# noahares/raxtax

Hardware: AMD Instinct MI355X
Metric: classified queries/sec (whole node) (higher is better)
Workload: dtype u32 bit-planes + f64

## Files before the change

raxtax_amd/csrc/rtx_emul.cpp:

```cpp
#include <algorithm>
#include <cmath>
#include <cstdint>
#include <cstring>
#include <array>
#include <vector>

#include "rtx_math.hpp"

using namespace rtx;

extern "C" {

uint32_t emul_planes_grouped(const uint32_t *rows, uint32_t n_rows, uint32_t groups, uint32_t *out) {
    constexpr int NP = 10;
    std::vector<std::array<uint32_t, NP>> part(groups);
    for (auto &p : part) p.fill(0);
    for (uint32_t u = 0; u + 8 * groups <= n_rows; u += 8 * groups)
        for (uint32_t g = 0; g < groups; g++) {
            const uint32_t *r = rows + u + 8 * g;
            uint32_t pl[NP];
            for (int p = 0; p < NP; p++) pl[p] = part[g][p];
            planes_ripple<NP, 3>(pl, planes_tree8<NP>(pl, r[0], r[1], r[2], r[3], r[4], r[5], r[6], r[7]));
            for (int p = 0; p < NP; p++) part[g][p] = pl[p];
        }
// ... 445 lines not shown
void emul_prune_threshold(uint32_t t, uint64_t n_refs, const uint32_t *hm_in, const double *lf, uint32_t tab_tmax, uint32_t *u_out,
                          uint32_t *i1_out) {
    emul_prune_threshold_x(t, n_refs, hm_in, lf, tab_tmax, 0, nullptr, nullptr, u_out, i1_out);
}
void emul_prune_threshold_tiles(uint32_t t, uint64_t n_refs, const uint32_t *hm_in, const double *lf, uint32_t tab_tmax, uint32_t ntiles,
                                const uint16_t *tile_ub, uint32_t *u_out, uint32_t *i1_out) {
    const uint32_t per = (ntiles + 63u) / 64u, ng = (ntiles + per - 1u) / per;
    std::vector<uint32_t> gub(ng, 0);
    std::vector<uint64_t> gn(ng, 0);
    for (uint32_t T = 0; T < ntiles; T++) {
        const uint32_t g = T / per;
        gub[g] = std::max<uint32_t>(gub[g], tile_ub[T]);
        const uint64_t lo = (uint64_t)T * 8192u, hi = std::min<uint64_t>(lo + 8192u, n_refs);
        gn[g] += hi > lo ? hi - lo : 0u;
    }
    emul_prune_threshold_x(t, n_refs, hm_in, lf, tab_tmax, ng, gub.data(), gn.data(), u_out, i1_out);
}

void emul_ref_slot(uint32_t r, uint32_t stride_bytes, uint32_t *word, uint32_t *bit) { ref_slot(r, stride_bytes, *word, *bit); }
uint32_t emul_slot_ref(uint32_t tile, uint32_t lane, uint32_t g, uint32_t j, uint32_t stride_bytes) {
    return tile * 8192u + (g * tile_lanes(stride_bytes, tile) + lane) * 8u + j;
}

void emul_merge_bytes(const uint32_t *sb, uint32_t *st) {
    st[0] += (sb[0] & 0xFFu) | ((sb[0] & 0xFF00u) << 8);
    st[1] += ((sb[0] >> 16) & 0xFFu) | ((sb[0] >> 24) << 16);
    st[2] += (sb[1] & 0xFFu) | ((sb[1] & 0xFF00u) << 8);
    st[3] += ((sb[1] >> 16) & 0xFFu) | ((sb[1] >> 24) << 16);
}

void emul_transpose64(const unsigned long long *in, unsigned long long *out) {
    unsigned long long x[64], y[64];
    for (int l = 0; l < 64; l++) x[l] = in[l];
    for (int s = 32; s >= 1; s >>= 1) {
        const unsigned long long m = s == 32 ? 0x00000000FFFFFFFFull : s == 16 ? 0x0000FFFF0000FFFFull : s == 8 ? 0x00FF00FF00FF00FFull
                                   : s == 4 ? 0x0F0F0F0F0F0F0F0Full : s == 2 ? 0x3333333333333333ull : 0x5555555555555555ull;
        for (int l = 0; l < 64; l++) y[l] = x[l ^ s];
        for (int l = 0; l < 64; l++) x[l] = (l & s) ? (((y[l] >> s) & m) | (x[l] & ~m)) : ((x[l] & m) | ((y[l] & m) << s));
    }
    for (int l = 0; l < 64; l++) out[l] = x[l];
}

uint32_t emul_finalise_rows(uint32_t n, uint32_t D, const uint8_t *k, const uint32_t *depth, const uint32_t *size, double n_total, uint32_t *rank,
                            double *local) {
    const uint32_t kw = (D + 3u) / 4u;
    std::vector<uint32_t> words((size_t)n * kw, 0u);
    for (uint32_t r = 0; r < n; r++)
        for (uint32_t w = 0; w < kw; w++) {
            uint32_t v = 0;
            for (uint32_t b = 0; b < 4u; b++) {
                const uint32_t d = 4u * w + b;
                v |= (uint32_t)(d < depth[r] && d < D ? k[(size_t)r * D + d] : 0u) << (8u * b);
            }
            words[(size_t)r * kw + w] = fin_be32(v);
        }
    uint32_t disagree = 0;
    for (uint32_t r = 0; r < n; r++) {
        uint32_t before = 0;
        for (uint32_t x = 0; x < n; x++) {
            const bool a = x != r && fin_row_before(k + (size_t)x * D, depth[x], x, k + (size_t)r * D, depth[r], r);
            const bool b = x != r && fin_row_before_words(&words[(size_t)x * kw], depth[x], x, &words[(size_t)r * kw], depth[r], r, kw);
            disagree += a != b;
            before += b ? 1u : 0u;
        }
        rank[r] = before;
        double eb[64];
        const uint32_t s0 = fin_node_expected(size + (size_t)r * D, depth[r], n_total, eb);
        const uint8_t *kr = k + (size_t)r * D;
        local[r] = fin_local_signal([&](uint32_t d) { return kr[d]; }, eb, s0, depth[r]);
    }
    return disagree;
}

int64_t emul_text_numbers(const double *v, uint64_t n, uint32_t n_hund, char *out, uint64_t cap) {
    TextWindow w{out, 0, 0, cap};
    for (uint64_t i = 0; i < n; i++) { text_put_fix5(w, v[i]); w.put('\n'); }
    for (uint32_t k = 0; k < n_hund; k++) { text_put_hund(w, k); w.put('\n'); }
    return w.pos > cap ? -1 : (int64_t)w.pos;
}

int64_t emul_text_batch(const char *lin_bytes, const uint64_t *lin_off, const uint8_t *lin_depth, const uint32_t *row_lineage,
                        const uint8_t *row_depth, const uint8_t *row_hund, const double *row_local, uint32_t D, uint64_t nq,
                        const char *labels, const uint64_t *label_off, const uint8_t *status, const uint64_t *row_begin,
                        const uint32_t *row_count, const double *gs, const uint32_t *one, const uint8_t *seq, const uint64_t *seq_off,
                        int tsv, char *out, uint64_t cap, uint64_t *out_off) {
    const TextSrc t{lin_bytes, lin_off, lin_depth, row_lineage, row_depth, row_hund, row_local, D};
    TextWindow w{out, 0, 0, cap};
    for (uint64_t q = 0; q < nq; q++) {
        out_off[q] = w.pos;
        const uint64_t n_out = status[q] != 0 || row_count[q] == 0 ? 0 : (one[q] != kTextNoOverride ? 1 : row_count[q]);
        for (uint64_t i = 0; i < n_out; i++) {
            if (i) w.put('\n');
            const TextRow r = text_row(t, labels + label_off[q], label_off[q + 1] - label_off[q], row_begin[q], i, one[q], gs[q]);
            if (tsv) {
                const uint8_t *sq = seq + seq_off[q];
                text_tsv_row(w, r, seq_off[q + 1] - seq_off[q], [&](uint64_t j) { return sq[j]; });
            } else {
                text_out_row(w, r);
            }
        }
        w.put('\0');
    }
    out_off[nq] = w.pos;
    return w.pos > cap ? -1 : (int64_t)w.pos;
}

uint32_t emul_nearest_scan(const void *lo, const uint16_t *hi, uint32_t in_tile, uint32_t peak, int packed) {
    const uint32_t per = packed ? 16u : 8u;
    for (uint32_t step = 0; nearest_lane_base(step, 0u, per) < in_tile; step++) {
        uint32_t mask[64];
        for (uint32_t lane = 0; lane < 64u; lane++) {
            const uint32_t b0 = nearest_lane_base(step, lane, per);
            mask[lane] = 0;
            if (b0 >= in_tile) continue;
            uint32_t w[4];
            if (packed) {
                std::memcpy(w, static_cast<const uint8_t *>(lo) + b0, 16);
                uint32_t h2;
                std::memcpy(&h2, hi + (b0 >> 3), 4);
                mask[lane] = nearest_match16(w, h2, peak, b0, in_tile);
            } else {
                std::memcpy(w, static_cast<const uint16_t *>(lo) + b0, 16);
                mask[lane] = nearest_match8(w, peak, b0, in_tile);
            }
        }
        for (uint32_t lane = 0; lane < 64u; lane++)
            if (mask[lane]) return nearest_lane_base(step, lane, per) + (uint32_t)__builtin_ctz(mask[lane]);
    }
    return 0xFFFFFFFFu;
}
void emul_packed_count_pos(uint32_t rl, uint32_t *byte, uint32_t *hi_word, uint32_t *hi_shift) { packed_count_pos(rl, *byte, *hi_word, *hi_shift); }

void emul_profile(uint64_t nq, const uint8_t *status, const uint32_t *row_count, const uint64_t *row_begin, const uint32_t *row_node,
                  const uint8_t *row_depth, const uint8_t *row_hund, uint32_t D, const uint32_t *parent, const uint8_t *node_depth,
                  const uint32_t *ref_leaf, uint32_t n_nodes, uint32_t n_refs, const uint32_t *one, uint32_t cutoff, uint64_t *clade,
                  uint64_t *direct, uint64_t *conf_sum, uint64_t *totals) {
    const ProfileSrc src{status, row_count, reinterpret_cast<const unsigned long long *>(row_begin), row_node, row_depth, row_hund, D, parent, node_depth, ref_leaf, n_nodes, n_refs};
    for (uint64_t q = 0; q < nq; q++) {
        const ProfileStep st = profile_step(src, q, one[q], cutoff);
        totals[0]++;
        totals[st.kind == kProfClassified ? 1 : (st.kind == kProfUnclassified ? 2 : 3)]++;
        if (st.kind != kProfClassified) continue;
        uint32_t node = st.node;
        for (uint32_t d = st.L; d-- > 0u;) {
            if (node >= n_nodes) break;
            clade[node]++;
            conf_sum[node] += st.at(d);
            if (d + 1u == st.L) direct[node]++;
            node = parent[node];
        }
    }
}

}
```

raxtax_amd/csrc/rtx_math.hpp:

```cpp
#pragma once

#include <cmath>
#include <cstdint>

#if defined(__HIPCC__)
#define RTX_HD __host__ __device__ __forceinline__
#else
#define RTX_HD inline
#endif

namespace rtx {


RTX_HD uint32_t tile_lanes(uint32_t stride_bytes, uint32_t tile) {
    const uint32_t rem = stride_bytes - tile * 1024u;
    return rem >= 1024u ? 64u : rem >> 4;
}
RTX_HD size_t bitmap_word(uint32_t row, uint32_t word, uint32_t n_rows1) {
    return ((size_t)(word >> 8) * n_rows1 + row) * 256u + (word & 255u);
}
RTX_HD void ref_slot(uint32_t r, uint32_t stride_bytes, uint32_t &word, uint32_t &bit) {
    const uint32_t tile = r >> 13, rl = r & 8191u;
    const uint32_t L = tile_lanes(stride_bytes, tile);
    const uint32_t c = rl >> 3, l = c % L, g = c / L;
// ... 185 lines not shown
        hi1 |= spread4(pl[p] >> (8 * b + 4)) << (p - 8);
    }
}

RTX_HD uint32_t byte_perm(uint32_t hi, uint32_t lo, uint32_t sel) {
#if defined(__HIP_DEVICE_COMPILE__)
    return __builtin_amdgcn_perm(hi, lo, sel);
#else
    const uint64_t v = ((uint64_t)hi << 32) | lo;
    uint32_t r = 0;
    for (int k = 0; k < 4; k++) {
        const uint32_t s = (sel >> (8 * k)) & 0xFFu;
        if (s < 8u) r |= (uint32_t)((v >> (8 * s)) & 0xFFu) << (8 * k);
    }
    return r;
#endif
}

RTX_HD void delta_swap_regs(uint32_t &a, uint32_t &b, int s, uint32_t m) {
    const uint32_t na = (a & m) | ((b & m) << s), nb = ((a >> s) & m) | (b & ~m);
    a = na;
    b = nb;
}
template <int NP>
RTX_HD void planes_unpack32(const uint32_t (&pl)[NP], uint32_t (&lo)[4][2]) {
    static_assert(NP >= 8, "at least eight planes");
    uint32_t r[8];
#pragma unroll
    for (int p = 0; p < 8; p++) r[p] = pl[p];
#pragma unroll
    for (int p = 0; p < 4; p++) delta_swap_regs(r[p], r[p + 4], 4, 0x0F0F0F0Fu);
#pragma unroll
    for (int p = 0; p < 8; p++)
        if (!(p & 2)) delta_swap_regs(r[p], r[p + 2], 2, 0x33333333u);
#pragma unroll
    for (int p = 0; p < 8; p += 2) delta_swap_regs(r[p], r[p + 1], 1, 0x55555555u);
#pragma unroll
    for (int h = 0; h < 2; h++) {
        const uint32_t x0 = byte_perm(r[4 * h + 1], r[4 * h], 0x05010400u), x1 = byte_perm(r[4 * h + 1], r[4 * h], 0x07030602u);
        const uint32_t y0 = byte_perm(r[4 * h + 3], r[4 * h + 2], 0x05010400u), y1 = byte_perm(r[4 * h + 3], r[4 * h + 2], 0x07030602u);
        lo[0][h] = byte_perm(y0, x0, 0x05040100u);
        lo[1][h] = byte_perm(y0, x0, 0x07060302u);
        lo[2][h] = byte_perm(y1, x1, 0x05040100u);
        lo[3][h] = byte_perm(y1, x1, 0x07060302u);
    }
}
template <int NP>
RTX_HD void planes_unpack8_hi(const uint32_t (&pl)[NP], int b, uint32_t &hi0, uint32_t &hi1) {
    hi0 = 0;
    hi1 = 0;
#pragma unroll
    for (int p = 8; p < NP; p++) {
        hi0 |= spread4(pl[p] >> (8 * b)) << (p - 8);
        hi1 |= spread4(pl[p] >> (8 * b + 4)) << (p - 8);
    }
}

struct PmfState {
    double v;
    double c;
    int k;
};

constexpr double kScaleLn = 354.89135644669199;
constexpr double kScaleUp = 1.2676506002282294e30;
constexpr double kScaleDown = 7.458340731200207e-155;

RTX_HD double ln_binom_tab(const double *lf, uint32_t n, uint32_t k) { return lf[n] - lf[k] - lf[n - k]; }

RTX_HD PmfState pmf_start(const double *lf, uint32_t t, uint32_t n, uint32_t m, double ln_total) {
    double x0 = ln_binom_tab(lf, t - m + n - 1, n) - ln_total;
    PmfState s;
    s.k = 0;
    if (x0 < -600.0) {
        s.k = (int)ceil((-600.0 - x0) / kScaleLn);
        x0 += (double)s.k * kScaleLn;
    }
    s.v = exp(x0);
    s.c = s.v;
    return s;
}

RTX_HD double ln_pmf_tab(const double *lf, uint32_t t, uint32_t n, uint32_t m, uint32_t i, double ln_total);
RTX_HD PmfState pmf_start_at(const double *lf, uint32_t t, uint32_t n, uint32_t m, uint32_t i_s, double ln_total) {
    double x0 = ln_pmf_tab(lf, t, n, m, i_s, ln_total);
    PmfState s;
    s.k = 0;
    if (x0 < -600.0) {
        s.k = (int)ceil((-600.0 - x0) / kScaleLn);
        x0 += (double)s.k * kScaleLn;
    }
    s.v = exp(x0);
    s.c = s.v;
    return s;
}

RTX_HD double pow_uint(double c, uint32_t h) {
    double r = 1.0, b = c;
    while (h) {
        if (h & 1u) r *= b;
        b *= b;
        h >>= 1;
    }
    return r;
}

RTX_HD double pmf_cmf_pow(const PmfState &s, uint32_t h) {
    if (s.k > 0 || !(s.c > 0.0)) return 0.0;
    return pow_uint(s.c, h);
}

struct InvDiv {
    RTX_HD double operator[](uint32_t x) const { return 1.0 / (double)x; }
};
template <class Inv>
RTX_HD void pmf_step(PmfState &s, const Inv &inv, uint32_t t, uint32_t n, uint32_t m, uint32_t i) {
    const double ratio = ((double)(m + i - 1) * inv[i]) * ((double)(n - i + 1) * inv[t - m + n - i]);
    s.v *= ratio;
    s.c += s.v;
    if (s.k > 0 && s.v > kScaleUp) {
        s.v *= kScaleDown;
        s.c *= kScaleDown;
        s.k -= 1;
    }
}

RTX_HD double neg_inf() { return -INFINITY; }

RTX_HD double pmf_ln_cmf(const PmfState &s) {
    if (s.k > 0 || !(s.c > 0.0)) return neg_inf();
    return log(s.c);
}

constexpr double kLnNegligibleP = -100.0;
constexpr double kLnTailSkip = -41.446531673892822;

RTX_HD double ln_pmf_tab(const double *lf, uint32_t t, uint32_t n, uint32_t m, uint32_t i, double ln_total) {
    return ln_binom_tab(lf, m + i - 1, i) + ln_binom_tab(lf, t - m + n - i - 1, n - i) - ln_total;
}

RTX_HD bool group_negligible(const double *lf, uint32_t t, uint32_t n, uint32_t m_hi, uint32_t i_lo, double ln_total) {
    if (i_lo == 0) return false;
    const double up = (double)(m_hi + i_lo - 1) * (double)(n - i_lo + 1);
    const double dn = (double)i_lo * (double)(t - m_hi + n - i_lo);
    if (!(up < dn)) return false;
    return log((double)(n - i_lo + 1)) + ln_pmf_tab(lf, t, n, m_hi, i_lo, ln_total) < kLnTailSkip;
}

constexpr double kPruneEpsHD = 1e-10;
constexpr double kPruneLnEpsHD = -23.025850929940457;
constexpr double kPruneHalfEpsHD = 0.5e-10;
constexpr uint32_t kPruneFarGap = 40;
constexpr uint32_t kPruneMaxNear = 12;

template <class WAf, class WBf>
RTX_HD void prune_window_sums(const double *lf, const double *inv, uint32_t t, uint32_t n, uint32_t m, uint32_t i1, double ln_total,
                              WAf wa, WBf wb, double &sa, double &sb) {
    sa = 0.0;
    sb = 0.0;
    const bool ok = m != 0u && m < t;
    const uint32_t ms = ok ? m : 1u;
    double x0 = ln_pmf_tab(lf, t, n, ms, i1, ln_total);
    if (x0 < -700.0) x0 = -700.0;
    double P = ok ? exp(x0) : 0.0;
    for (uint32_t l = 0; l < 64u && i1 + l <= n; l++) {
        sa += P * wa(l);
        sb += P * wb(l);
        const uint32_t i = i1 + l;
        if (i < n) P *= ((double)(ms + i) * inv[i + 1u]) * ((double)(n - i) * inv[t - ms + n - i - 1u]);
    }
}

RTX_HD double only_last_pmf_tab(const double *lf, uint32_t t, uint32_t n, uint32_t m, double ln_total) {
    if (m == t) return 1.0;
    if (m == 0) return 0.0;
    return exp(ln_binom_tab(lf, m + n - 1, n) - ln_total);
}

RTX_HD bool fin_row_before(const uint8_t *kx, uint32_t dx, uint32_t ix, const uint8_t *ky, uint32_t dy, uint32_t iy) {
    const uint32_t n = dx < dy ? dx : dy;
    for (uint32_t d = 0; d < n; d++)
        if (kx[d] != ky[d]) return kx[d] > ky[d];
    if (dx != dy) return dx > dy;
    return ix < iy;
}
RTX_HD bool fin_row_before_words(const uint32_t *kx, uint32_t dx, uint32_t ix, const uint32_t *ky, uint32_t dy, uint32_t iy, uint32_t kw) {
    for (uint32_t w = 0; w < kw; w++)
        if (kx[w] != ky[w]) return kx[w] > ky[w];
    if (dx != dy) return dx > dy;
    return ix < iy;
}
RTX_HD uint32_t fin_be32(uint32_t v) { return (v >> 24) | ((v >> 8) & 0xFF00u) | ((v << 8) & 0xFF0000u) | (v << 24); }

RTX_HD uint32_t fin_node_expected(const uint32_t *size, uint32_t depth, double n_total, double *eb) {
#if defined(__clang__)
#pragma clang fp contract(off)
#endif
    if (depth == 0) return 0;
    uint32_t s0 = depth - 1u;
    for (uint32_t d = 0; d < depth; d++)
        if (1.0 > (double)size[d] / n_total) { s0 = d; break; }
    double b_sum = 0.0;
    for (uint32_t d = s0; d < depth; d++) b_sum += (double)size[d] / n_total;
    for (uint32_t d = 0; d < depth; d++) eb[d] = d < s0 ? 0.0 : ((double)size[d] / n_total) / b_sum;
    return s0;
}
template <class K>
RTX_HD double fin_local_signal(K k, const double *eb, uint32_t s0, uint32_t depth) {
#if defined(__clang__)
#pragma clang fp contract(off)
#endif
    if (depth == 0) return 0.0;
    double a_sum = 0.0;
    for (uint32_t d = s0; d < depth; d++) a_sum += (double)k(d) / 100.0;
    double s = 0.0;
    for (uint32_t d = s0; d < depth; d += 4u) {
        double e[4];
#pragma unroll
        for (uint32_t u = 0; u < 4u; u++) e[u] = d + u < depth ? eb[d + u] : 0.0;
#pragma unroll
        for (uint32_t u = 0; u < 4u; u++) {
            if (d + u < depth) {
                const double x = ((double)k(d + u) / 100.0) / a_sum - e[u];
                const double xx = x * x;
                s = s + xx;
            }
        }
    }
    return sqrt(s);
}

struct TextCount {
    uint64_t pos = 0;
    RTX_HD void put(char) { pos++; }
    template <class F>
    RTX_HD void put_gen(uint64_t n, F) { pos += n; }
};
struct TextWindow {
    char *buf;
    uint64_t pos, w0, w1;
    RTX_HD void put(char c) {
        if (pos >= w0 && pos < w1) buf[pos - w0] = c;
        pos++;
    }
    template <class F>
    RTX_HD void put_gen(uint64_t n, F f) {
        const uint64_t lo = pos > w0 ? pos : w0, hi = pos + n < w1 ? pos + n : w1;
        for (uint64_t i = lo; i < hi; i++) buf[i - w0] = f(i - pos);
        pos += n;
    }
};

template <class S>
RTX_HD void text_put_u64(S &s, uint64_t v) {
    uint32_t nd = 1;
    for (uint64_t p = 10; nd < 20 && v >= p; p *= 10) nd++;
    uint64_t div = 1;
    for (uint32_t i = 1; i < nd; i++) div *= 10;
    for (uint32_t i = 0; i < nd; i++) {
        s.put((char)('0' + v / div % 10));
        div /= 10;
    }
}

template <class S>
RTX_HD void text_put_big_int(S &s, double v) {
    int e2 = 0;
    const double fr = frexp(v, &e2);
    uint64_t m = (uint64_t)ldexp(fr, 53);
    const int sh = e2 - 53;
    uint32_t limb[34] = {0};
    const int w = sh / 32, b = sh % 32;
    limb[w] = (uint32_t)(m << b);
    limb[w + 1] = (uint32_t)(m >> (32 - b));
    limb[w + 2] = b ? (uint32_t)(m >> (64 - b)) : 0u;
    uint32_t chunk[40];
    int nc = 0, top = 33;
    while (top >= 0) {
        while (top >= 0 && limb[top] == 0) top--;
        if (top < 0) break;
        uint64_t rem = 0;
        for (int i = top; i >= 0; i--) {
            const uint64_t cur = rem << 32 | limb[i];
            limb[i] = (uint32_t)(cur / 1000000000u);
            rem = cur % 1000000000u;
        }
        chunk[nc++] = (uint32_t)rem;
    }
    text_put_u64(s, chunk[nc - 1]);
    for (int i = nc - 2; i >= 0; i--)
        for (uint32_t d = 100000000u; d; d /= 10) s.put((char)('0' + chunk[i] / d % 10));
}

template <class S>
RTX_HD void text_put_fix5(S &s, double v) {
    const bool neg = std::signbit(v);
    if (std::isnan(v)) { if (neg) s.put('-'); s.put('n'); s.put('a'); s.put('n'); return; }
    if (neg) s.put('-');
    if (std::isinf(v)) { s.put('i'); s.put('n'); s.put('f'); return; }
    const double a = fabs(v);
    double I = floor(a);
    const double F = a - I;
    const double p = F * 1e5, e = fma(F, 1e5, -p);
    const double n = floor(p), f = p - n;
    bool up = false;
    if (f >= 0.25) {
// ... 150 lines not shown
```

raxtax_amd/csrc/rtx_prune.hip:

```cpp
#include <hip/hip_runtime.h>

#include "rtx_kernels.hpp"
#include "rtx_math.hpp"
#include "rtx_wave.hpp"

namespace rtx {

static constexpr double kPruneLnEps = kPruneLnEpsHD;
static constexpr double kPruneHalfEps = kPruneHalfEpsHD;
#ifndef RTX_PRUNE_WAVES
#define RTX_PRUNE_WAVES 4
#endif
#ifndef RTX_PRUNE_TURNS
#define RTX_PRUNE_TURNS 16
#endif
static constexpr uint32_t kPruneWavesPerBlock = 4;

__device__ __forceinline__ uint32_t wave_max_u32p(uint32_t v) { return wave_max_u32(v); }

__global__ __launch_bounds__(64 * kPruneWavesPerBlock, RTX_PRUNE_WAVES) void prune_kernel(PruneParams p, ProbTables tb) {
    extern __shared__ double prune_lds[];
    for (uint32_t i = threadIdx.x; i < p.nlf; i += 64u * kPruneWavesPerBlock) prune_lds[i] = p.lnfact[i];
    __syncthreads();
    const uint32_t lane = threadIdx.x & 63u, pair = blockIdx.x * kPruneWavesPerBlock + (threadIdx.x >> 6);
    if (pair * 2u >= p.nq) return;
    uint16_t *ub_lds = reinterpret_cast<uint16_t *>(prune_lds + p.nlf) + (size_t)(threadIdx.x >> 6) * 2u * p.ntiles;
    const double *lf = prune_lds;
    const double ln_n = log((double)p.n_total);
    uint32_t thr[2] = {0u, 0u};
    uint32_t ist_prev = 0;
    unsigned long long st[8] = {0, 0, 0, 0, 0, 0, 0, 0};
    const bool has_b = pair * 2u + 1u < p.nq;
    for (uint32_t x = 0; x < 2u; x++) {
        if (x == 1u && !has_b) break;
        const uint32_t q = pair * 2u + x;
        for (uint32_t T = lane; T < p.ntiles; T += 64) ub_lds[x * p.ntiles + T] = p.tile_ub[(size_t)q * p.tile_ub_stride + T];
        const uint32_t bkey = p.best_key[q];
        uint32_t ub_best = bkey >> 20;
        const uint32_t bb = 0xFFFFFu - (bkey & 0xFFFFFu);
        uint32_t M = 0;
        uint32_t hm = 0;
        if (p.phase == 2u) {
            const uint32_t *bq = p.best + (size_t)q * kPruneBestWords;
            ub_best = bq[0];
            hm = bq[2u + lane];
            M = wave_max_u32p(hm);
        } else if (p.cbitmap) {
            static_assert(kPruneShift == 6, "a block of the block-major bitmap is the block of the bounds");
            const uint32_t nr = p.nrows[q];
            const uint32_t *rows = p.rows + (size_t)q * p.rstride;
            const uint32_t zero_row = p.n_rows1 - 1u;
            const uint32_t nr_pad = (nr + 63u) & ~63u;
            const uint2 *C = p.cbitmap + (size_t)bb * p.n_rows1;
            uint32_t pl[2][11];
#pragma unroll
            for (int w = 0; w < 2; w++)
#pragma unroll
                for (int b = 0; b < 11; b++) pl[w][b] = 0;
            for (uint32_t i0 = 0; i0 < nr_pad; i0 += 256u) {
                uint32_t id[4];
                uint2 v[4];
#pragma unroll
                for (int k = 0; k < 4; k++) {
                    const uint32_t i = i0 + (uint32_t)k * 64u + lane;
                    id[k] = i < nr_pad ? rows[i] : zero_row;
                }
#pragma unroll
                for (int k = 0; k < 4; k++) v[k] = C[id[k]];
#pragma unroll
                for (int k = 0; k < 4; k++) {
                    uint32_t cx = v[k].x, cy = v[k].y;
#pragma unroll
                    for (int b = 0; b < 6; b++) {
                        const uint32_t nx = pl[0][b] & cx, ny = pl[1][b] & cy;
                        pl[0][b] ^= cx;
                        pl[1][b] ^= cy;
                        cx = nx;
                        cy = ny;
                    }
                }
            }
            uint32_t r[11];
            {
                const bool up = (lane & 32u) != 0u;
                uint32_t o[11];
#pragma unroll
                for (int b = 0; b < 11; b++) {
                    r[b] = up ? pl[1][b] : pl[0][b];
                    o[b] = (uint32_t)__shfl_xor((int)(up ? pl[0][b] : pl[1][b]), 32, 64);
                }
                planes_add<11>(r, o);
            }
#pragma unroll
            for (int d = 16; d >= 1; d >>= 1) {
                uint32_t o[11];
#pragma unroll
                for (int b = 0; b < 11; b++) o[b] = (uint32_t)__shfl_xor((int)r[b], d, 64);
                planes_add<11>(r, o);
            }
            uint32_t cnt = 0;
#pragma unroll
            for (int b = 0; b < 11; b++) cnt |= ((r[b] >> (lane & 31u)) & 1u) << b;
            const uint64_t rr = ((uint64_t)bb << kPruneShift) + (uint64_t)lane;
            bool ok = rr < p.n_refs;
            if (p.flags & RTX_SKIP_EXACT_MATCHES) {
                const uint64_t qin = p.perm[p.q0 + q];
                uint64_t xe0 = 0, xe1 = 0;
                const uint32_t *xids = nullptr;
                exact_range(p.exact, qin, xe0, xe1, xids);
                for (uint64_t e = xe0; e < xe1; e++) ok = ok && (uint64_t)(xids[e] - p.ref_base) != rr;
            }
            hm = ok ? cnt : 0u;
            M = wave_max_u32p(hm);
        } else {
            constexpr uint32_t kChunks = (1u << kPruneShift) / 8u;
            const uint32_t nr = p.nrows[q];
            const uint32_t *rows = p.rows + (size_t)q * p.rstride;
            const uint64_t qin = p.perm[p.q0 + q];
            uint64_t xe0 = 0, xe1 = 0;
            const uint32_t *xids = nullptr;
            if (p.flags & RTX_SKIP_EXACT_MATCHES) exact_range(p.exact, qin, xe0, xe1, xids);
            const uint32_t zero_row = p.n_rows1 - 1u;
            constexpr uint32_t kRowsPerTurn = 64u / kChunks;
            const uint32_t ch = lane & (kChunks - 1u), rg = lane / kChunks;
            uint32_t word, bit;
            {
                const uint64_t r0 = ((uint64_t)bb << kPruneShift) + (uint64_t)ch * 8u;
                ref_slot((uint32_t)(r0 < p.n_refs ? r0 : (uint64_t)bb << kPruneShift), p.stride_bytes, word, bit);
            }
            static_assert(kChunks == 8u, "the byte counters of the best block's exact counts hold the rows of one lane in eight (blocks of 64 references)");
            uint32_t acc_lo = 0u, acc_hi = 0u;
            uint32_t acc[4] = {0u, 0u, 0u, 0u};
            const uint32_t bit4 = bit + 4u;
            const uint32_t nr_pad = (nr + 63u) & ~63u;
            constexpr uint32_t kTurns = RTX_PRUNE_TURNS, kPiece = kTurns * kRowsPerTurn;
            static_assert(kPiece % 64u == 0u && kPiece <= 128u, "a piece of the row list = one or two loads per lane");
            auto load_ids = [&](uint32_t i0, uint32_t (&id)[2]) {
#pragma unroll
                for (uint32_t k = 0; k < kPiece / 64u; k++) {
                    const uint32_t i = i0 + k * 64u + lane;
                    id[k] = i < nr_pad ? rows[i] : zero_row;
                }
            };
            uint32_t id[2] = {zero_row, zero_row}, idn[2] = {zero_row, zero_row};
            load_ids(0, id);
            for (uint32_t i0 = 0; i0 < nr; i0 += kPiece) {
                if (i0 + kPiece < nr) load_ids(i0 + kPiece, idn);
                uint32_t w[kTurns];
#pragma unroll
                for (uint32_t u = 0; u < kTurns; u++) {
                    const uint32_t e = u * kRowsPerTurn + rg;
                    const uint32_t row = (uint32_t)__shfl((int)id[e >> 6], (int)(e & 63u), 64);
                    w[u] = p.bitmap[bitmap_word(row, word, p.n_rows1)];
                }
#pragma unroll
                for (uint32_t u = 0; u < kTurns; u++) {
                    acc_lo += __umul24((w[u] >> bit) & 0xFu, 0x204081u) & 0x01010101u;
                    acc_hi += __umul24((w[u] >> bit4) & 0xFu, 0x204081u) & 0x01010101u;
                }
                id[0] = idn[0];
                id[1] = idn[1];
                acc[0] += (acc_lo & 0xFFu) | ((acc_lo & 0xFF00u) << 8);
                acc[1] += ((acc_lo >> 16) & 0xFFu) | ((acc_lo >> 24) << 16);
                acc[2] += (acc_hi & 0xFFu) | ((acc_hi & 0xFF00u) << 8);
                acc[3] += ((acc_hi >> 16) & 0xFFu) | ((acc_hi >> 24) << 16);
                acc_lo = 0u;
                acc_hi = 0u;
            }
#pragma unroll
            for (int k = 0; k < 4; k++)
#pragma unroll
                for (uint32_t d = 32; d >= kChunks; d >>= 1) acc[k] += (uint32_t)__shfl_xor((int)acc[k], (int)d, 64);
            {
                const uint32_t c = lane >> 3, j = lane & 7u;
                const uint32_t v0 = (uint32_t)__shfl((int)acc[0], (int)c, 64), v1 = (uint32_t)__shfl((int)acc[1], (int)c, 64),
                               v2 = (uint32_t)__shfl((int)acc[2], (int)c, 64), v3 = (uint32_t)__shfl((int)acc[3], (int)c, 64);
                const uint32_t vv = (j & 4u) ? ((j & 2u) ? v3 : v2) : ((j & 2u) ? v1 : v0);
                const uint32_t cnt = (vv >> ((j & 1u) * 16u)) & 0xFFFFu;
                const uint64_t r = ((uint64_t)bb << kPruneShift) + (uint64_t)lane;
                bool ok = lane < (1u << kPruneShift) && r < p.n_refs;
                if (p.flags & RTX_SKIP_EXACT_MATCHES)
                    for (uint64_t e = xe0; e < xe1; e++) ok = ok && (uint64_t)(xids[e] - p.ref_base) != r;
                hm = ok ? cnt : 0u;
                M = wave_max_u32p(hm);
            }
        }
        if (p.detail) p.detail[(size_t)q * kPruneDetailWords + 8u + lane] = hm;
        if (p.phase == 1u) {
            uint32_t *bq = p.best + (size_t)q * kPruneBestWords;
            bq[2u + lane] = hm;
            if (lane == 0) { bq[0] = ub_best; bq[1] = 0u; }
            continue;
        }
        const uint32_t t = p.t[q], n = t >> 1;
        uint32_t u_max = 0, i1_q = 0;
        if (t >= 16u && t <= tb.tmax && M >= 1u && n >= 2u) {
            const double ln_total = ln_binom_tab(lf, t + n - 1, n);
            if (M >= t) {
                uint32_t mine = 0;
                for (uint32_t u = 1u + lane; u < t; u += 64)
                    if (ln_binom_tab(lf, u + n - 1, n) - ln_total + ln_n <= kPruneLnEps) mine = u;
                u_max = wave_max_u32p(mine);
            } else {
                const double *Ct = tb.cmf + tb.off[t];
                if (hm * 5u < M * 4u) hm = 0u;
                const double n_h = (double)__popcll(__ballot(hm != 0u));
                const uint32_t h_min = 0xFFFFFFFFu - wave_max_u32p(hm ? 0xFFFFFFFFu - hm : 0u);
                const double ln_f_lo = log(n_h + (double)p.n_total), ln_f_hi = log(n_h + (double)p.n_total * (double)(n - 1u));
                auto passes = [&](uint32_t i) -> bool {
                    const double v = hm ? Ct[(size_t)hm * (n + 1) + i] : 0.0;
                    const double sum = wave_sum_f64_dpp(v);
                    if (sum + ln_f_hi <= kPruneLnEps) return true;
                    if (sum + ln_f_lo > kPruneLnEps) return false;
                    return sum + log(n_h + (double)p.n_total * (double)(i + 1u)) <= kPruneLnEps;
                };
                uint32_t ist1 = 0;
                if (passes(0u)) {
                    uint32_t g;
                    if (x == 1u && ist_prev) g = ist_prev - 1u;
                    else {
                        const double pm = (double)M / (double)t;
                        const double mu = (double)n * pm, sd = sqrt((double)n * pm * (1.0 - pm) * (double)(t + n) / (double)(t + 1u));
                        const double gg = mu - 6.0 * sd;
                        g = gg > 0.0 ? (uint32_t)gg : 0u;
                    }
                    g = g > n - 2u ? n - 2u : g;
                    uint32_t lo, hi;
                    if (passes(g)) {
                        lo = g;
                        uint32_t step = 1u;
                        while (lo + step <= n - 2u && passes(lo + step)) { lo += step; step <<= 1; }
                        hi = lo + step <= n - 2u ? lo + step : n - 1u;
                    } else {
                        hi = g;
                        uint32_t step = 1u;
                        while (hi > step && !passes(hi - step)) { hi -= step; step <<= 1; }
                        lo = hi > step ? hi - step : 0u;
                    }
                    while (hi - lo > 1u) {
                        const uint32_t mid = (lo + hi) >> 1;
                        if (passes(mid)) lo = mid; else hi = mid;
                    }
                    ist1 = lo + 1u;
                }
                ist_prev = ist1;
                if (ist1) {
                    const uint32_t i1 = ist1;
                    const double ln_len = log((double)(n - i1 + 1u));
                    uint32_t first_fail = h_min;
                    for (uint32_t u = 1u + lane; u < h_min; u += 64) {
                        const double up = (double)(u + i1) * (double)(n - i1), dn = (double)(i1 + 1u) * (double)(t - u + n - i1 - 1u);
                        if (!(up < dn && ln_len + ln_pmf_tab(lf, t, n, u, i1, ln_total) + ln_n <= kPruneLnEps)) first_fail = u < first_fail ? u : first_fail;
                    }
                    first_fail = 0xFFFFFFFFu - wave_max_u32p(0xFFFFFFFFu - first_fail);
                    u_max = first_fail - 1u;
                    i1_q = i1;
                    {
                        const bool tile_aware = p.phase == 0u;
                        uint32_t gub = 0;
                        double gnd = 0.0;
                        {
                            const uint32_t per = (p.ntiles + 63u) >> 6;
                            for (uint32_t k = 0; k < per; k++) {
                                const uint32_t T = lane * per + k;
                                if (T < p.ntiles) {
                                    const uint32_t b = ub_lds[x * p.ntiles + T];
                                    gub = b > gub ? b : gub;
                                    const uint64_t lo = (uint64_t)T * 8192u, hi = lo + 8192u < p.n_refs ? lo + 8192u : p.n_refs;
                                    gnd += (double)(hi - lo);
                                }
                            }
                        }
                        const double kept = tile_aware ? wave_sum_f64_dpp(gub > u_max ? gnd : 0.0) : (double)p.n_total;
                        const double ln_kept = log(kept > 1.0 ? kept : 1.0);
                        const uint32_t iw = i1 + lane;
                        const bool tail_pt = lane == 63u;
                        const bool vi = iw <= n;
                        double lnG = 0.0;
                        unsigned long long hb = __ballot(hm != 0u);
                        const uint32_t iwc = vi ? iw : n;
                        while (hb) {
                            double v[4];
#pragma unroll
                            for (int k = 0; k < 4; k++) {
                                v[k] = 0.0;
                                if (hb) {
                                    const int h = __builtin_ctzll(hb);
                                    hb &= hb - 1ull;
                                    const uint32_t m = (uint32_t)__builtin_amdgcn_readlane((int)hm, h);
                                    v[k] = Ct[(size_t)m * (n + 1) + iwc];
                                }
                            }
#pragma unroll
                            for (int k = 0; k < 4; k++) lnG += v[k];
                        }
                        const double gw = vi && !tail_pt ? exp(lnG) : 0.0;
                        const double ww = vi && !tail_pt ? exp(fmin(0.0, ln_kept + lnG)) : 0.0;
                        const double incl = wave_incl_scan_f64_dpp(ww);
                        const double a_tot = readlane_f64(incl, 63);
                        const double len_tail = vi ? (double)(n - iw + 1u) : 0.0;
                        const double WA = tail_pt ? len_tail * (a_tot + 1.0) : (vi ? incl - ww : 0.0);
                        const double WB = tail_pt ? len_tail : gw;
                        const double nn = (double)p.n_total;
                        const bool has_tail = i1 + 63u <= n;
                        auto sums_at = [&](uint32_t m, double &a, double &b) {
                            const double P = vi && m != 0u ? exp(ln_pmf_tab(lf, t, n, m, iw, ln_total)) : 0.0;
                            a = wave_sum_f64_dpp(P * WA);
                            b = wave_sum_f64_dpp(P * WB);
                        };
                        double gsa = 0.0, gsb = 0.0, far_a = 0.0, far_b = 0.0, n_far = 0.0, mid_a = 0.0, mid_b = 0.0, n_mid = 0.0;
                        bool near = false;
                        if (tile_aware) {
                            const uint32_t m_far = u_max > kPruneFarGap ? u_max - kPruneFarGap : 0u;
                            near = gnd > 0.0 && gub > u_max;
                            const bool mid = gnd > 0.0 && gub > m_far && gub <= u_max;
                            unsigned long long nb = __ballot(near);
                            if ((uint32_t)__popcll(nb) > kPruneMaxNear) {
                                near = gnd > 0.0;
                                const uint32_t gcap = gub < h_min ? gub : h_min - 1u;
                                prune_window_sums(lf, p.inv, t, n, gcap, i1, ln_total, [&](uint32_t l) { return readlane_f64(WA, (int)l); },
                                                  [&](uint32_t l) { return readlane_f64(WB, (int)l); }, gsa, gsb);
                            } else {
                                n_far = wave_sum_f64_dpp(near || mid ? 0.0 : gnd);
                                n_mid = wave_sum_f64_dpp(mid ? gnd : 0.0);
                                if (m_far) sums_at(m_far, far_a, far_b);
                                if (n_mid > 0.0) sums_at(u_max, mid_a, mid_b);
                                while (nb) {
                                    const int g = __builtin_ctzll(nb);
                                    nb &= nb - 1ull;
                                    const uint32_t m = (uint32_t)__builtin_amdgcn_readlane((int)gub, g);
                                    double a, b;
                                    sums_at(m < h_min ? m : h_min - 1u, a, b);
                                    if ((int)lane == g) { gsa = a; gsb = b; }
                                }
                            }
                        }
                        auto crit = [&](uint32_t u) -> bool {
                            bool falling = true;
                            if (has_tail) {
                                const uint32_t j = i1 + 63u;
                                falling = (double)(u + j) * (double)(n - j) < (double)(j + 1u) * (double)(t - u + n - j - 1u);
                            }
                            double a, b;
                            sums_at(u, a, b);
                            if (!tile_aware) return falling && nn * a <= kPruneHalfEps && nn * b <= kPruneHalfEps;
                            const bool dead = gub <= u;
                            return falling && wave_sum_f64_dpp(near ? gnd * (dead ? gsa : a) : 0.0) + n_far * far_a + n_mid * mid_a <= kPruneHalfEps &&
                                   wave_sum_f64_dpp(near ? gnd * (dead ? gsb : b) : 0.0) + n_far * far_b + n_mid * mid_b <= kPruneHalfEps;
                        };
                        uint32_t lo = u_max, hi = h_min - 1u;
                        while (lo < hi) {
                            const uint32_t mid = (lo + hi + 1u) >> 1;
                            if (crit(mid)) lo = mid; else hi = mid - 1u;
                        }
                        u_max = lo;
                    }
                }
            }
        }
        thr[x] = u_max;
        if (lane == 0) { p.thr_out[q] = (uint16_t)u_max; p.i1_out[q] = (uint16_t)(u_max ? i1_q : 0u); }
        if (p.detail && lane == 0) {
            uint32_t *d = p.detail + (size_t)q * kPruneDetailWords;
            d[0] = bb; d[1] = M; d[2] = u_max; d[3] = u_max ? i1_q : 0u; d[4] = ub_best; d[5] = t; d[6] = 0u; d[7] = 0u;
        }
        st[2] += M; st[3] += u_max; st[4] += ub_best; st[5] += 1ull;
        if (ub_best < M) st[6] += 1ull;
    }
    if (p.phase == 1u) return;
    __builtin_amdgcn_fence(__ATOMIC_ACQ_REL, "wavefront");
    __builtin_amdgcn_wave_barrier();
    unsigned long long dead_refs[2] = {0, 0};
    uint32_t n_live = 0, n_qlive = 0;
    uint32_t n_rec[2] = {0u, 0u};
    for (uint32_t T0 = 0; T0 < p.ntiles; T0 += 64) {
        const uint32_t T = T0 + lane;
        bool la = false, lb = false;
        if (T < p.ntiles) {
            la = thr[0] == 0u || (uint32_t)ub_lds[T] > thr[0];
            lb = has_b && (thr[1] == 0u || (uint32_t)ub_lds[p.ntiles + T] > thr[1]);
        }
        const unsigned long long ba = __ballot(la), bb2 = __ballot(lb);
        if (lane == 0) {
            uint32_t *wa = p.live + (size_t)(pair * 2u) * p.live_words, *wb = wa + p.live_words;
            wa[T0 >> 5] = (uint32_t)ba;
            if ((T0 >> 5) + 1u < p.live_words) wa[(T0 >> 5) + 1u] = (uint32_t)(ba >> 32);
            if (has_b) {
                wb[T0 >> 5] = (uint32_t)bb2;
                if ((T0 >> 5) + 1u < p.live_words) wb[(T0 >> 5) + 1u] = (uint32_t)(bb2 >> 32);
            }
        }
        if (T < p.ntiles) {
            const uint64_t lo = (uint64_t)T * 8192u, hi = lo + 8192u < p.n_refs ? lo + 8192u : p.n_refs;
            if (!la) dead_refs[0] += hi - lo;
            if (!lb) dead_refs[1] += hi - lo;
        }
        if (p.rec.nslots) {
            const unsigned long long lt = (1ull << lane) - 1ull;
            const uint32_t ka = n_rec[0] + (uint32_t)__popcll(ba & lt), kb = n_rec[1] + (uint32_t)__popcll(bb2 & lt);
            if (la && ka < kRecMaxSlots) p.rec.slots[(size_t)(pair * 2u) * kRecMaxSlots + ka] = (uint16_t)T;
            if (lb && kb < kRecMaxSlots) p.rec.slots[(size_t)(pair * 2u + 1u) * kRecMaxSlots + kb] = (uint16_t)T;
            n_rec[0] += (uint32_t)__popcll(ba);
            n_rec[1] += (uint32_t)__popcll(bb2);
        }
        n_live += (uint32_t)__popcll(ba | bb2);
        n_qlive += (uint32_t)__popcll(ba) + (uint32_t)__popcll(bb2);
    }
    if (p.rec.nslots) {
        const uint32_t cap = p.rec_max_slots < kRecMaxSlots ? p.rec_max_slots : kRecMaxSlots;
        const bool ra = thr[0] != 0u && n_rec[0] != 0u && n_rec[0] <= cap, rb = has_b && thr[1] != 0u && n_rec[1] != 0u && n_rec[1] <= cap;
        if (lane < kRecMaxSlots) {
            p.rec.cnt[(size_t)(pair * 2u) * kRecMaxSlots + lane] = 0u;
            if (has_b) p.rec.cnt[(size_t)(pair * 2u + 1u) * kRecMaxSlots + lane] = 0u;
        }
        if (lane == 0) {
            p.rec.nslots[pair * 2u] = (uint16_t)(ra ? n_rec[0] : 0u);
            if (has_b) p.rec.nslots[pair * 2u + 1u] = (uint16_t)(rb ? n_rec[1] : 0u);
            if (p.cnt_row) {
                auto row_for = [&](bool records) -> uint32_t {
                    if (records) return 0xFFFFFFFFu;
                    const uint32_t r = atomicAdd(p.cnt_cursor, 1u);
                    if (r < p.cnt_cap) return r;
                    atomicOr(p.flags_out, 4u);
                    return 0xFFFFFFFFu;
                };
                p.cnt_row[pair * 2u] = row_for(ra);
                if (has_b) p.cnt_row[pair * 2u + 1u] = row_for(rb);
            }
        }
    }
#pragma unroll
    for (int d = 32; d >= 1; d >>= 1) { dead_refs[0] += __shfl_xor(dead_refs[0], d, 64); dead_refs[1] += __shfl_xor(dead_refs[1], d, 64); }
    if (lane == 0) {
// ... 41 lines not shown
```

Measured before the change: 13.01 million.

## Process both queries of a pair abreast with batched 8-way threshold search

```diff
diff --git a/raxtax_amd/csrc/rtx_emul.cpp b/raxtax_amd/csrc/rtx_emul.cpp
--- a/raxtax_amd/csrc/rtx_emul.cpp
+++ b/raxtax_amd/csrc/rtx_emul.cpp
@@ -621,4 +621,40 @@
     }
 }
 
-}
+uint32_t emul_batched_search(uint32_t n_max, uint32_t guess, int32_t b, uint32_t *info) {
+    uint32_t rounds = 0, asked = 0, c_min = 0xFFFFFFFFu, c_max = 0, outside = 0;
+    const uint32_t r = batched_search(n_max, guess, [&](const uint32_t (&c)[kSearchK], uint32_t cnt) {
+        uint32_t mask = 0;
+        rounds++;
+        for (uint32_t k = 0; k < cnt; k++) {
+            asked++;
+            c_min = std::min(c_min, c[k]);
+            c_max = std::max(c_max, c[k]);
+            outside += c[k] > n_max;
+            if ((int64_t)c[k] <= (int64_t)b) mask |= 1u << k;
+        }
+        return mask;
+    });
+    info[0] = rounds; info[1] = asked; info[2] = c_min; info[3] = c_max; info[4] = outside;
+    return r;
+}
+uint64_t emul_batched_search_grid(uint32_t n_lo, uint32_t n_hi, uint64_t *worst) {
+    uint64_t bad = 0, runs = 0;
+    uint32_t w_rounds = 0, w_asked = 0;
+    for (uint32_t n_max = n_lo; n_max <= n_hi; n_max++)
+        for (int32_t b = -1; b <= (int32_t)n_max; b++) {
+            const int64_t gs[7] = {0, b, (int64_t)b - 1, (int64_t)b + 1, (int64_t)b - 40, (int64_t)b + 40, (int64_t)n_max};
+            for (int64_t g : gs) {
+                uint32_t info[5];
+                const uint32_t r = emul_batched_search(n_max, (uint32_t)std::max<int64_t>(g, 0), b, info);
+                bad += r != (uint32_t)(b + 1) || info[4] != 0u;
+                w_rounds = std::max(w_rounds, info[0]);
+                w_asked = std::max(w_asked, info[1]);
+                runs++;
+            }
+        }
+    worst[0] = w_rounds; worst[1] = w_asked; worst[2] = runs;
+    return bad;
+}
+
+}
diff --git a/raxtax_amd/csrc/rtx_math.hpp b/raxtax_amd/csrc/rtx_math.hpp
--- a/raxtax_amd/csrc/rtx_math.hpp
+++ b/raxtax_amd/csrc/rtx_math.hpp
@@ -361,6 +361,62 @@
 constexpr double kPruneHalfEpsHD = 0.5e-10;
 constexpr uint32_t kPruneFarGap = 40;
 constexpr uint32_t kPruneMaxNear = 12;
+
+constexpr uint32_t kSearchK = 8;
+struct BatchedSearch {
+    uint32_t lo1;
+    uint32_t hi;
+    uint32_t g;
+    uint32_t n_max;
+    bool first;
+    RTX_HD void start(uint32_t n_max_, uint32_t guess) {
+        lo1 = 0u;
+        hi = n_max_ + 1u;
+        n_max = n_max_;
+        g = guess < n_max_ ? guess : n_max_;
+        first = true;
+    }
+    RTX_HD bool done() const { return lo1 >= hi; }
+    RTX_HD uint32_t result() const { return lo1; }
+    RTX_HD uint32_t candidates(uint32_t (&c)[kSearchK]) const {
+        if (first) {
+            const uint32_t down[3] = {32u, 8u, 2u};
+            c[0] = 0u;
+#pragma unroll
+            for (uint32_t k = 0; k < 3u; k++) {
+                c[1u + k] = g > down[k] ? g - down[k] : 0u;
+                c[7u - k] = n_max - g > down[k] ? g + down[k] : n_max;
+            }
+            c[4] = g;
+            return kSearchK;
+        }
+        const uint32_t m = hi - lo1;
+#pragma unroll
+        for (uint32_t k = 0; k < kSearchK; k++)
+            c[k] = m <= kSearchK ? lo1 + (k < m ? k : m - 1u) : lo1 + ((k + 1u) * (m + 1u)) / (kSearchK + 1u) - 1u;
+        return m <= kSearchK ? m : kSearchK;
+    }
+    RTX_HD void update(const uint32_t (&c)[kSearchK], uint32_t cnt, uint32_t pass_mask) {
+#pragma unroll
+        for (uint32_t k = 0; k < kSearchK; k++) {
+            if (k >= cnt) continue;
+            if ((pass_mask >> k) & 1u) lo1 = c[k] + 1u > lo1 ? c[k] + 1u : lo1;
+            else hi = c[k] < hi ? c[k] : hi;
+        }
+        first = false;
+    }
+};
+template <class F>
+RTX_HD uint32_t batched_search(uint32_t n_max, uint32_t guess, F passes_many) {
+    BatchedSearch s;
+    s.start(n_max, guess);
+    while (!s.done()) {
+        uint32_t c[kSearchK];
+        const uint32_t cnt = s.candidates(c);
+        s.update(c, cnt, passes_many(c, cnt));
+    }
+    return s.result();
+}
 
 template <class WAf, class WBf>
 RTX_HD void prune_window_sums(const double *lf, const double *inv, uint32_t t, uint32_t n, uint32_t m, uint32_t i1, double ln_total,
diff --git a/raxtax_amd/csrc/rtx_prune.hip b/raxtax_amd/csrc/rtx_prune.hip
--- a/raxtax_amd/csrc/rtx_prune.hip
+++ b/raxtax_amd/csrc/rtx_prune.hip
@@ -11,12 +11,55 @@
 #ifndef RTX_PRUNE_WAVES
 #define RTX_PRUNE_WAVES 4
 #endif
+#ifndef RTX_PRUNE_ABREAST
+#define RTX_PRUNE_ABREAST 7
+#endif
 #ifndef RTX_PRUNE_TURNS
 #define RTX_PRUNE_TURNS 16
 #endif
+#ifndef RTX_PRUNE_WINDOW_ROWS
+#define RTX_PRUNE_WINDOW_ROWS 16
+#endif
+static constexpr int kWinRows = RTX_PRUNE_WINDOW_ROWS;
 static constexpr uint32_t kPruneWavesPerBlock = 4;
 
 __device__ __forceinline__ uint32_t wave_max_u32p(uint32_t v) { return wave_max_u32(v); }
+
+__device__ __forceinline__ uint32_t block_planes_reduce(const uint32_t (&pl)[2][11], uint32_t lane) {
+    uint32_t r[11];
+    {
+        const bool up = (lane & 32u) != 0u;
+        uint32_t o[11];
+#pragma unroll
+        for (int b = 0; b < 11; b++) {
+            r[b] = up ? pl[1][b] : pl[0][b];
+            o[b] = (uint32_t)__shfl_xor((int)(up ? pl[0][b] : pl[1][b]), 32, 64);
+        }
+        planes_add<11>(r, o);
+    }
+#pragma unroll
+    for (int d = 16; d >= 1; d >>= 1) {
+        uint32_t o[11];
+#pragma unroll
+        for (int b = 0; b < 11; b++) o[b] = (uint32_t)__shfl_xor((int)r[b], d, 64);
+        planes_add<11>(r, o);
+    }
+    uint32_t cnt = 0;
+#pragma unroll
+    for (int b = 0; b < 11; b++) cnt |= ((r[b] >> (lane & 31u)) & 1u) << b;
+    return cnt;
+}
+__device__ __forceinline__ void block_planes_add_row(uint32_t (&pl)[2][11], uint2 v) {
+    uint32_t cx = v.x, cy = v.y;
+#pragma unroll
+    for (int b = 0; b < 6; b++) {
+        const uint32_t nx = pl[0][b] & cx, ny = pl[1][b] & cy;
+        pl[0][b] ^= cx;
+        pl[1][b] ^= cy;
+        cx = nx;
+        cy = ny;
+    }
+}
 
 __global__ __launch_bounds__(64 * kPruneWavesPerBlock, RTX_PRUNE_WAVES) void prune_kernel(PruneParams p, ProbTables tb) {
     extern __shared__ double prune_lds[];
@@ -31,16 +74,216 @@
     uint32_t ist_prev = 0;
     unsigned long long st[8] = {0, 0, 0, 0, 0, 0, 0, 0};
     const bool has_b = pair * 2u + 1u < p.nq;
+#if RTX_PRUNE_ABREAST
+    const bool abreast = p.phase == 0u && p.cbitmap != nullptr;
+#else
+    const bool abreast = false;
+#endif
+    uint32_t pre_hm0 = 0u, pre_hm1 = 0u;
+    uint32_t pre_M[2] = {0u, 0u}, pre_ub[2] = {0u, 0u}, pre_bb[2] = {0u, 0u}, pre_ist1[2] = {0u, 0u};
+    double pre_lnG0 = 0.0, pre_lnG1 = 0.0;
+    if (abreast) {
+        static_assert(kPruneShift == 6, "a block of the block-major bitmap is the block of the bounds");
+        const bool val[2] = {true, has_b};
+        const uint32_t zero_row = p.n_rows1 - 1u;
+        uint32_t tq[2], nr_pad[2];
+        uint64_t toff[2];
+        const uint32_t *rows[2];
+        const uint2 *C[2];
+#pragma unroll
+        for (uint32_t x = 0; x < 2u; x++) {
+            const uint32_t q = pair * 2u + x;
+            uint32_t bkey = 0xFFFFFu, nr = 0u;
+            tq[x] = 0u;
+            if (val[x]) {
+                for (uint32_t T = lane; T < p.ntiles; T += 64) ub_lds[x * p.ntiles + T] = p.tile_ub[(size_t)q * p.tile_ub_stride + T];
+                bkey = p.best_key[q];
+                nr = p.nrows[q];
+                tq[x] = p.t[q];
+            }
+            toff[x] = tq[x] >= 16u && tq[x] <= tb.tmax ? tb.off[tq[x]] : 0ull;
+            pre_ub[x] = bkey >> 20;
+            pre_bb[x] = 0xFFFFFu - (bkey & 0xFFFFFu);
+            nr_pad[x] = (nr + 63u) & ~63u;
+            rows[x] = p.rows + (size_t)(val[x] ? q : pair * 2u) * p.rstride;
+            C[x] = p.cbitmap + (size_t)pre_bb[x] * p.n_rows1;
+        }
+        uint32_t pl[2][2][11];
+#pragma unroll
+        for (int x = 0; x < 2; x++)
+#pragma unroll
+            for (int w = 0; w < 2; w++)
+#pragma unroll
+                for (int b = 0; b < 11; b++) pl[x][w][b] = 0;
+#if RTX_PRUNE_ABREAST & 4
+        const uint32_t pad_max = nr_pad[0] > nr_pad[1] ? nr_pad[0] : nr_pad[1];
+        for (uint32_t i0 = 0; i0 < pad_max; i0 += 256u) {
+            uint32_t id[2][4];
+            uint2 v[2][4];
+#pragma unroll
+            for (int x = 0; x < 2; x++)
+#pragma unroll
+                for (int k = 0; k < 4; k++) {
+                    const uint32_t i = i0 + (uint32_t)k * 64u + lane;
+                    id[x][k] = i < nr_pad[x] ? rows[x][i] : zero_row;
+                }
+#pragma unroll
+            for (int x = 0; x < 2; x++)
+#pragma unroll
+                for (int k = 0; k < 4; k++) v[x][k] = C[x][id[x][k]];
+#pragma unroll
+            for (int x = 0; x < 2; x++)
+#pragma unroll
+                for (int k = 0; k < 4; k++) block_planes_add_row(pl[x], v[x][k]);
+        }
+#else
+#pragma unroll
+        for (int x = 0; x < 2; x++)
+            for (uint32_t i0 = 0; i0 < nr_pad[x]; i0 += 256u) {
+                uint32_t id[4];
+                uint2 v[4];
+#pragma unroll
+                for (int k = 0; k < 4; k++) {
+                    const uint32_t i = i0 + (uint32_t)k * 64u + lane;
+                    id[k] = i < nr_pad[x] ? rows[x][i] : zero_row;
+                }
+#pragma unroll
+                for (int k = 0; k < 4; k++) v[k] = C[x][id[k]];
+#pragma unroll
+                for (int k = 0; k < 4; k++) block_planes_add_row(pl[x], v[k]);
+            }
+#endif
+        uint32_t hmq[2] = {0u, 0u};
+#pragma unroll
+        for (uint32_t x = 0; x < 2u; x++) {
+            if (!val[x]) continue;
+            const uint32_t q = pair * 2u + x;
+            const uint32_t cnt = block_planes_reduce(pl[x], lane);
+            const uint64_t rr = ((uint64_t)pre_bb[x] << kPruneShift) + (uint64_t)lane;
+            bool ok = rr < p.n_refs;
+            if (p.flags & RTX_SKIP_EXACT_MATCHES) {
+                const uint64_t qin = p.perm[p.q0 + q];
+                uint64_t xe0 = 0, xe1 = 0;
+                const uint32_t *xids = nullptr;
+                exact_range(p.exact, qin, xe0, xe1, xids);
+                for (uint64_t e = xe0; e < xe1; e++) ok = ok && (uint64_t)(xids[e] - p.ref_base) != rr;
+            }
+            hmq[x] = ok ? cnt : 0u;
+            pre_M[x] = wave_max_u32p(hmq[x]);
+        }
+        pre_hm0 = hmq[0];
+        pre_hm1 = hmq[1];
+        BatchedSearch sr[2];
+        bool run[2] = {false, false};
+        const double *Ct[2] = {tb.cmf, tb.cmf};
+        uint32_t hmH[2] = {0u, 0u}, nn1[2] = {1u, 1u};
+        double n_h[2] = {0.0, 0.0}, ln_f_lo[2] = {0.0, 0.0}, ln_f_hi[2] = {0.0, 0.0};
+#pragma unroll
+        for (uint32_t x = 0; x < 2u; x++) {
+            const uint32_t t = tq[x], n = t >> 1, M = pre_M[x];
+            if (!(val[x] && t >= 16u && t <= tb.tmax && M >= 1u && n >= 2u && M < t)) continue;
+            Ct[x] = tb.cmf + toff[x];
+            nn1[x] = n + 1u;
+            hmH[x] = hmq[x] * 5u < M * 4u ? 0u : hmq[x];
+            n_h[x] = (double)__popcll(__ballot(hmH[x] != 0u));
+            ln_f_lo[x] = log(n_h[x] + (double)p.n_total);
+            ln_f_hi[x] = log(n_h[x] + (double)p.n_total * (double)(n - 1u));
+            const double pm = (double)M / (double)t;
+            const double mu = (double)n * pm, sd = sqrt((double)n * pm * (1.0 - pm) * (double)(t + n) / (double)(t + 1u));
+            const double gg = mu - 6.0 * sd;
+            sr[x].start(n - 2u, gg > 0.0 ? (uint32_t)gg : 0u);
+            run[x] = true;
+        }
+        while ((run[0] && !sr[0].done()) || (run[1] && !sr[1].done())) {
+            uint32_t c[2][kSearchK], cnt[2] = {0u, 0u};
+            double v[2][kSearchK];
+#pragma unroll
+            for (uint32_t x = 0; x < 2u; x++) {
+                if (!(run[x] && !sr[x].done())) continue;
+                cnt[x] = sr[x].candidates(c[x]);
+                const double *row = Ct[x] + (size_t)hmH[x] * nn1[x];
+#pragma unroll
+                for (uint32_t k = 0; k < kSearchK; k++) v[x][k] = k < cnt[x] && hmH[x] ? row[c[x][k]] : 0.0;
+            }
+#pragma unroll
+            for (uint32_t x = 0; x < 2u; x++) {
+                if (!cnt[x]) continue;
+                uint32_t mask = 0u, band = 0u, cv = 0u;
+                double sv = 0.0;
+#pragma unroll
+                for (uint32_t k = 0; k < kSearchK; k++) {
+                    if (k >= cnt[x]) continue;
+                    const double sum = wave_sum_f64_dpp(v[x][k]);
+                    const bool yes = sum + ln_f_hi[x] <= kPruneLnEps, no = sum + ln_f_lo[x] > kPruneLnEps;
+                    mask |= yes ? 1u << k : 0u;
+                    band |= yes || no ? 0u : 1u << k;
+                    sv = lane == k ? sum : sv;
+                    cv = lane == k ? c[x][k] : cv;
+                }
+                band = (uint32_t)__builtin_amdgcn_readfirstlane((int)band);
+                while (band) {
+                    const int k = __builtin_ctz(band);
+                    band &= band - 1u;
+                    const double sum = readlane_f64(sv, k);
+                    const uint32_t i = (uint32_t)__builtin_amdgcn_readlane((int)cv, k);
+                    if (sum + log(n_h[x] + (double)p.n_total * (double)(i + 1u)) <= kPruneLnEps) mask |= 1u << k;
+                }
+                sr[x].update(c[x], cnt[x], (uint32_t)__builtin_amdgcn_readfirstlane((int)mask));
+            }
+        }
+#pragma unroll
+        for (uint32_t x = 0; x < 2u; x++) pre_ist1[x] = run[x] ? sr[x].result() : 0u;
+#if RTX_PRUNE_ABREAST & 2
+        {
+            unsigned long long hb[2];
+            uint32_t iwc[2];
+            double lnG[2] = {0.0, 0.0};
+#pragma unroll
+            for (uint32_t x = 0; x < 2u; x++) {
+                const uint32_t n = nn1[x] - 1u, iw = pre_ist1[x] + lane;
+                iwc[x] = iw <= n ? iw : n;
+                hb[x] = pre_ist1[x] ? __ballot(hmH[x] != 0u) : 0ull;
+            }
+            while (hb[0] | hb[1]) {
+                double w[2][kWinRows];
+#pragma unroll
+                for (uint32_t x = 0; x < 2u; x++)
+#pragma unroll
+                    for (int k = 0; k < kWinRows; k++) {
+                        w[x][k] = 0.0;
+                        if (hb[x]) {
+                            const int h = __builtin_ctzll(hb[x]);
+                            hb[x] &= hb[x] - 1ull;
+                            const uint32_t m = (uint32_t)__builtin_amdgcn_readlane((int)hmH[x], h);
+                            w[x][k] = Ct[x][(size_t)m * nn1[x] + iwc[x]];
+                        }
+                    }
+#pragma unroll
+                for (uint32_t x = 0; x < 2u; x++)
+#pragma unroll
+                    for (int k = 0; k < kWinRows; k++) lnG[x] += w[x][k];
+            }
+            pre_lnG0 = lnG[0];
+            pre_lnG1 = lnG[1];
+        }
+#endif
+    }
     for (uint32_t x = 0; x < 2u; x++) {
         if (x == 1u && !has_b) break;
         const uint32_t q = pair * 2u + x;
-        for (uint32_t T = lane; T < p.ntiles; T += 64) ub_lds[x * p.ntiles + T] = p.tile_ub[(size_t)q * p.tile_ub_stride + T];
-        const uint32_t bkey = p.best_key[q];
-        uint32_t ub_best = bkey >> 20;
-        const uint32_t bb = 0xFFFFFu - (bkey & 0xFFFFFu);
+        uint32_t bkey = 0u;
+        if (!abreast) {
+            for (uint32_t T = lane; T < p.ntiles; T += 64) ub_lds[x * p.ntiles + T] = p.tile_ub[(size_t)q * p.tile_ub_stride + T];
+            bkey = p.best_key[q];
+        }
+        uint32_t ub_best = abreast ? (x ? pre_ub[1] : pre_ub[0]) : bkey >> 20;
+        const uint32_t bb = abreast ? (x ? pre_bb[1] : pre_bb[0]) : 0xFFFFFu - (bkey & 0xFFFFFu);
         uint32_t M = 0;
         uint32_t hm = 0;
-        if (p.phase == 2u) {
+        if (abreast) {
+            hm = x ? pre_hm1 : pre_hm0;
+            M = x ? pre_M[1] : pre_M[0];
+        } else if (p.phase == 2u) {
             const uint32_t *bq = p.best + (size_t)q * kPruneBestWords;
             ub_best = bq[0];
             hm = bq[2u + lane];
@@ -68,39 +311,9 @@
 #pragma unroll
                 for (int k = 0; k < 4; k++) v[k] = C[id[k]];
 #pragma unroll
-                for (int k = 0; k < 4; k++) {
-                    uint32_t cx = v[k].x, cy = v[k].y;
-#pragma unroll
-                    for (int b = 0; b < 6; b++) {
-                        const uint32_t nx = pl[0][b] & cx, ny = pl[1][b] & cy;
-                        pl[0][b] ^= cx;
-                        pl[1][b] ^= cy;
-                        cx = nx;
-                        cy = ny;
-                    }
-                }
-            }
-            uint32_t r[11];
-            {
-                const bool up = (lane & 32u) != 0u;
-                uint32_t o[11];
-#pragma unroll
-                for (int b = 0; b < 11; b++) {
-                    r[b] = up ? pl[1][b] : pl[0][b];
-                    o[b] = (uint32_t)__shfl_xor((int)(up ? pl[0][b] : pl[1][b]), 32, 64);
-                }
-                planes_add<11>(r, o);
-            }
-#pragma unroll
-            for (int d = 16; d >= 1; d >>= 1) {
-                uint32_t o[11];
-#pragma unroll
-                for (int b = 0; b < 11; b++) o[b] = (uint32_t)__shfl_xor((int)r[b], d, 64);
-                planes_add<11>(r, o);
-            }
-            uint32_t cnt = 0;
-#pragma unroll
-            for (int b = 0; b < 11; b++) cnt |= ((r[b] >> (lane & 31u)) & 1u) << b;
+                for (int k = 0; k < 4; k++) block_planes_add_row(pl, v[k]);
+            }
+            const uint32_t cnt = block_planes_reduce(pl, lane);
             const uint64_t rr = ((uint64_t)bb << kPruneShift) + (uint64_t)lane;
             bool ok = rr < p.n_refs;
             if (p.flags & RTX_SKIP_EXACT_MATCHES) {
@@ -206,42 +419,46 @@
                 if (hm * 5u < M * 4u) hm = 0u;
                 const double n_h = (double)__popcll(__ballot(hm != 0u));
                 const uint32_t h_min = 0xFFFFFFFFu - wave_max_u32p(hm ? 0xFFFFFFFFu - hm : 0u);
-                const double ln_f_lo = log(n_h + (double)p.n_total), ln_f_hi = log(n_h + (double)p.n_total * (double)(n - 1u));
-                auto passes = [&](uint32_t i) -> bool {
-                    const double v = hm ? Ct[(size_t)hm * (n + 1) + i] : 0.0;
-                    const double sum = wave_sum_f64_dpp(v);
-                    if (sum + ln_f_hi <= kPruneLnEps) return true;
-                    if (sum + ln_f_lo > kPruneLnEps) return false;
-                    return sum + log(n_h + (double)p.n_total * (double)(i + 1u)) <= kPruneLnEps;
-                };
                 uint32_t ist1 = 0;
-                if (passes(0u)) {
-                    uint32_t g;
-                    if (x == 1u && ist_prev) g = ist_prev - 1u;
-                    else {
-                        const double pm = (double)M / (double)t;
-                        const double mu = (double)n * pm, sd = sqrt((double)n * pm * (1.0 - pm) * (double)(t + n) / (double)(t + 1u));
-                        const double gg = mu - 6.0 * sd;
-                        g = gg > 0.0 ? (uint32_t)gg : 0u;
+                if (abreast) {
+                    ist1 = x ? pre_ist1[1] : pre_ist1[0];
+                } else {
+                    const double ln_f_lo = log(n_h + (double)p.n_total), ln_f_hi = log(n_h + (double)p.n_total * (double)(n - 1u));
+                    auto passes = [&](uint32_t i) -> bool {
+                        const double v = hm ? Ct[(size_t)hm * (n + 1) + i] : 0.0;
+                        const double sum = wave_sum_f64_dpp(v);
+                        if (sum + ln_f_hi <= kPruneLnEps) return true;
+                        if (sum + ln_f_lo > kPruneLnEps) return false;
+                        return sum + log(n_h + (double)p.n_total * (double)(i + 1u)) <= kPruneLnEps;
+                    };
+                    if (passes(0u)) {
+                        uint32_t g;
+                        if (x == 1u && ist_prev) g = ist_prev - 1u;
+                        else {
+                            const double pm = (double)M / (double)t;
+                            const double mu = (double)n * pm, sd = sqrt((double)n * pm * (1.0 - pm) * (double)(t + n) / (double)(t + 1u));
+                            const double gg = mu - 6.0 * sd;
+                            g = gg > 0.0 ? (uint32_t)gg : 0u;
+                        }
+                        g = g > n - 2u ? n - 2u : g;
+                        uint32_t lo, hi;
+                        if (passes(g)) {
+                            lo = g;
+                            uint32_t step = 1u;
+                            while (lo + step <= n - 2u && passes(lo + step)) { lo += step; step <<= 1; }
+                            hi = lo + step <= n - 2u ? lo + step : n - 1u;
+                        } else {
+                            hi = g;
+                            uint32_t step = 1u;
+                            while (hi > step && !passes(hi - step)) { hi -= step; step <<= 1; }
+                            lo = hi > step ? hi - step : 0u;
+                        }
+                        while (hi - lo > 1u) {
+                            const uint32_t mid = (lo + hi) >> 1;
+                            if (passes(mid)) lo = mid; else hi = mid;
+                        }
+                        ist1 = lo + 1u;
                     }
-                    g = g > n - 2u ? n - 2u : g;
-                    uint32_t lo, hi;
-                    if (passes(g)) {
-                        lo = g;
-                        uint32_t step = 1u;
-                        while (lo + step <= n - 2u && passes(lo + step)) { lo += step; step <<= 1; }
-                        hi = lo + step <= n - 2u ? lo + step : n - 1u;
-                    } else {
-                        hi = g;
-                        uint32_t step = 1u;
-                        while (hi > step && !passes(hi - step)) { hi -= step; step <<= 1; }
-                        lo = hi > step ? hi - step : 0u;
-                    }
-                    while (hi - lo > 1u) {
-                        const uint32_t mid = (lo + hi) >> 1;
-                        if (passes(mid)) lo = mid; else hi = mid;
-                    }
-                    ist1 = lo + 1u;
                 }
                 ist_prev = ist1;
                 if (ist1) {
@@ -279,6 +496,12 @@
                         double lnG = 0.0;
                         unsigned long long hb = __ballot(hm != 0u);
                         const uint32_t iwc = vi ? iw : n;
+#if RTX_PRUNE_ABREAST & 2
+                        if (abreast) {
+                            lnG = x ? pre_lnG1 : pre_lnG0;
+                            hb = 0ull;
+                        }
+#endif
                         while (hb) {
                             double v[4];
 #pragma unroll
```

New measurement: 12.79 million. 1.7% lower.
